# CliMA/ClimateParameterizations.jl

Hardware: AMD Instinct MI355X
Metric: column-timesteps/sec (fwd+adjoint), 32-level wind-mixing NDE (higher is better)
Workload: dtype f32

## Files before the change

### climateparameterizations.jl_amd/csrc/engine_regtile.hip

```cpp
#include <cstdlib>
#include "regtile_dev.h"
#include "kernel_select.h"

#ifndef RT16_WAVES
#define RT16_WAVES 8
#endif
#ifndef RT_ADJ_CH
#define RT_ADJ_CH 8
#endif
#define RT_TAPEZ (20 * 256)
#define RT_TAPE2 (20 * 256)

__host__ __device__ constexpr int rt16_q_net(int Q) { return Q < 36 ? Q / 12 : Q - 36; }
__host__ __device__ constexpr int rt16_q_quad(int Q) { return Q < 36 ? Q % 12 : 12; }
__host__ __device__ constexpr int rt16_q_slot(int n, int qq) { return qq < 12 ? 12 * n + qq : 36 + n; }

template <int ACT>
__device__ __forceinline__ void rt_mlp_forward(const float* wl, const RtBases& b, const f32x16 (&X)[3], int h, f32x16 (&O)[3]) {
    f32x16 A1[5];
#pragma unroll
    for (int mt = 0; mt < 5; mt++) {
        f32x16 acc;
#pragma unroll
        for (int r = 0; r < 16; r++) {
// ... 568 lines not shown
                            for (int G = 0; G < 24; G += 4) rt_act_pair4_at<ACT>(A1, D1, G);
                            rt_act_pair_at<ACT>(A1, D1, 24);
                        }
                    } else {
#pragma unroll
                        for (int t = 0; t < 2; t++) {
                            f32x16 acc;
#pragma unroll
                            for (int r = 0; r < 16; r++) acc[r] = (t * 16 + r < 25) ? wl[RT_B1C + n * 50 + 2 * (t * 16 + r) + h] : 0.0f;
                            const int base = a1n[t] + n * 50 * RT_LD1;
                            acc = rt_chain<48, RT_ADJ_CH>(wl, acc, [=](int k) { return base + (k >> 4) * 32 + RHO0(k & 15); },
                                                          [&](int k) { return X[k >> 4][k & 15]; });
#pragma unroll
                            for (int r = 0; r < 16; r++) {
                                float av = 0.0f, dv = 0.0f;
                                if (t * 16 + r < 25) rt_act_pair<ACT>(acc[r], av, dv);
                                A1[t][r] = av;
                                D1[t][r] = dv;
                            }
                        }
                    }
                    RT_STAMP(1);
                    f32x16 Z2;
                    {
                        f32x16 acc;
#pragma unroll
                        for (int r = 0; r < 16; r++) acc[r] = r < 10 ? wl[RT_B2C + n * 20 + 2 * r + h] : 0.0f;
                        const int base2 = a2b + n * 20 * RT_LD2;
                        Z2 = rt_chain<25, 5>(wl, acc, [=](int k) { return base2 + 2 * k; },
                                             [&](int k) { return A1[k >> 4][k & 15]; });
                    }
                    RT_STAMP(2);
                    {
                        f32x16 TA;
                        if (EARLY3 && n == 0) TA = TA3;
                        else { TA = rt_transpose(tb, dOn, wbase, rbase); b3acc[n] += rt_sum16(TA); }
                        f32x16 A2;
#pragma unroll
                        for (int r = 0; r < 16; r += 4) {
                            f32x2v a0 = {0.0f, 0.0f}, d0 = {0.0f, 0.0f}, a1 = {0.0f, 0.0f}, d1 = {0.0f, 0.0f};
                            if (r < 8) rt_act_pair4<ACT>((f32x2v){Z2[r], Z2[r + 1]}, (f32x2v){Z2[r + 2], Z2[r + 3]}, a0, d0, a1, d1);
                            else if (r == 8) rt_act_pair2<ACT>((f32x2v){Z2[8], Z2[9]}, a0, d0);
                            A2[r] = a0.x; A2[r + 1] = a0.y; A2[r + 2] = a1.x; A2[r + 3] = a1.y;
                            Z2[r] = d0.x; Z2[r + 1] = d0.y; Z2[r + 2] = d1.x; Z2[r + 3] = d1.y;
                        }
                        const f32x16 TB = rt_transpose(tb, A2, wbase, rbase);
                        gW3[n] = rt_outer(gW3[n], TA, TB);
                    }
                    {
                        const int base = b3T + n * 31 * RT_LD3;
                        f32x16 da;
                        if (EARLY3 && n == 0) da = da3;
                        else da = rt_chain<16, 8>(wl, (f32x16)(0.0f), [=](int k) { return base + RHO0(k) * RT_LD3; },
                                                  [&](int k) { return dOn[k]; });
#pragma unroll
                        for (int r = 0; r < 16; r++) Z2[r] = da[r] * Z2[r];
                    }
                    RT_STAMP(3);
                    if (ZT && n < 2) load_z1(step, st, n + 1, A1n);
                    u32x4 Lr[9];
                    const u32x4* lg = nullptr;
                    if constexpr (SPLIT) {
                        int lz = lane;
                        asm volatile("" : "+v"(lz));
                        lg = reinterpret_cast<const u32x4*>(wimg + RT_ASIMG_OFF + RT_ASIMG_L) + n * 9 * 64 + lz;
#pragma unroll
                        for (int u = 0; u < 3; u++) Lr[u] = lg[u * 64];
                    }
                    {
                        const f32x16 TA = rt_transpose(tb, Z2, wbase, rbase);
                        b2acc[n] += rt_sum16(TA);
#pragma unroll
                        for (int t = 0; t < 2; t++) {
                            const f32x16 TB = rt_transpose(tb, A1[t], wbase, rbase);
                            gW2[n][t] = rt_outer(gW2[n][t], TA, TB);
                        }
                    }
                    RT_STAMP(4);
#pragma unroll
                    for (int t = 0; t < 2; t++) {
                        const int base = b2T[t] + n * 20 * RT_LD2;
                        const f32x16 da = rt_chain<10, 10>(wl, (f32x16)(0.0f), [=](int k) { return base + 2 * k * RT_LD2; },
                                                           [&](int k) { return Z2[k]; });
#pragma unroll
                        for (int r = 0; r < 16; r++) D1[t][r] = da[r] * D1[t][r];
                    }
                    auto store_delta = [&] {
#pragma unroll
                    for (int g = 0; g < 25; g++) {
                        const int G = 25 * n + g;
                        if ((G & 3) == 0 && g + 3 < 25) {
                            const f32x4v v = {D1[g >> 4][g & 15], D1[(g + 1) >> 4][(g + 1) & 15], D1[(g + 2) >> 4][(g + 2) & 15],
                                              D1[(g + 3) >> 4][(g + 3) & 15]};
                            RT_NT_STORE4(dst + (G >> 2) * 256, v);
                        }
                    }
                    if (n == 0) carry[0] = D1[1][8];
                    if (n == 1) {
                        RT_NT_STORE4(dst + 6 * 256, ((f32x4v){carry[0], D1[0][0], D1[0][1], D1[0][2]}));
                        carry[0] = D1[1][7];
                        carry[1] = D1[1][8];
                    }
                    if (n == 2) {
                        RT_NT_STORE4(dst + 12 * 256, ((f32x4v){carry[0], carry[1], D1[0][0], D1[0][1]}));
                        RT_NT_STORE4(dst + 18 * 256, ((f32x4v){D1[1][6], D1[1][7], D1[1][8], 0.0f}));
                    }
                    };
                    if constexpr (!SPLIT) store_delta();
                    RT_STAMP(5);
                    if (ZT && n < 2) __builtin_amdgcn_sched_barrier(0);
                    if constexpr (SPLIT) {
                        const u32x4* hm = reinterpret_cast<const u32x4*>(rt_smem) + lane;
#pragma unroll
                        for (int c = 0; c < 3; c++) {
                            if (c < 2) {
#pragma unroll
                                for (int u = 0; u < 3; u++) Lr[3 * (c + 1) + u] = lg[(3 * (c + 1) + u) * 64];
                            }
                            float d8[8];
#pragma unroll
                            for (int u = 0; u < 8; u++) d8[u] = D1[(8 * c + u) >> 4][(8 * c + u) & 15];
                            const Bf3 Bc = bf3_split8(d8);
#pragma unroll
                            for (int q = 0; q < 3; q++) {
                                const int G = n * 9 + c * 3 + q, slot = c * 3 + q;
                                const u32x4 Ah = hm[(G * 2) * 64], Am = hm[(G * 2 + 1) * 64];
                                if (ZT && n < 2 && slot >= 2) {
                                    if (slot == 2) z1_stamp(n);
                                    if (slot < 8) rt_act_pair4_at<ACT>(A1n, D1n, 4 * (slot - 2));
                                    else rt_act_pair_at<ACT>(A1n, D1n, 24);
                                }
                                xb[q] = mfma_bf(Am, Bc.m, xb[q]);
                                xb[q] = mfma_bf(Ah, Bc.l, xb[q]);
                                xb[q] = mfma_bf(Am, Bc.h, xb[q]);
                                xb[q] = mfma_bf(Ah, Bc.m, xb[q]);
                                xb[q] = mfma_bf(Ah, Bc.h, xb[q]);
                                xb[q] = mfma_bf(Lr[slot], Bc.h, xb[q]);
                                RT_SCHED_FENCE();
                            }
                        }
                        const float* left = rt_smem + RT_ASIMG_LEFT + (n * 2 + h) * 96 + i_;
#pragma unroll
                        for (int q = 0; q < 3; q++) xb[q] = mfma32(left[q * 32], D1[1][8], xb[q]);
                        store_delta();
                    } else
#pragma unroll
                    for (int q = 0; q < 3; q++) {
                        const int base = b1T + q * 32 + n * 50 * RT_LD1;
                        xb[q] = rt_chain_fill<25, 5>(wl, xb[q], [=](int g) { return base + 2 * g * RT_LD1; },
                                                     [&](int g) { return D1[g >> 4][g & 15]; },
                                                     [&](int c) {
                                                         if (ZT && n < 2 && (q > 0 || c > 0)) {
                                                             if (q * 5 + c == 2) z1_stamp(n);
#pragma unroll
                                                             for (int G = 0; G < 24; G += 4)
                                                                 if ((G >> 2) * 2 + 2 == q * 5 + c)
                                                                     rt_act_pair4_at<ACT>(A1n, D1n, G);
                                                             if (q * 5 + c == 14) rt_act_pair_at<ACT>(A1n, D1n, 24);
                                                         }
                                                     });
                    }
                    if (ZT && n < 2) {
#pragma unroll
                        for (int t = 0; t < 2; t++) { A1[t] = A1n[t]; D1[t] = D1n[t]; }
                    }
                }
                RT_STAMP(6);
#pragma unroll
                for (int q = 0; q < 3; q++) xbs[q] += xb[q];
            }
#pragma unroll
            for (int q = 0; q < 3; q++) {
#pragma unroll
                for (int r = 0; r < 16; r++) lam[RT_LAM(q * 16 + r, lane)] += xbs[q][r];
                xbs[q] = (f32x16)(0.0f);
            }
        }
    }

#ifndef COLNDE_STAMPS_FWD
    RT_STAMP_FLUSH();
#endif
    float* out = slab + (size_t)tile * (m.n_params + 8);
    const int r_j = (j & 3) + 4 * (j >> 3), h_j = (j >> 2) & 1;
#pragma unroll
    for (int n = 0; n < 3; n++) {
        if (r_j < 10) {
            const int f2 = 2 * r_j + h_j;
#pragma unroll
            for (int r = 0; r < 16; r++) {
                const int face = RHO0(r) + 4 * h;
                if (face >= 1) out[n * m.net_size + m.w_off[2] + f2 * 31 + face - 1] = gW3[n][r];
            }
        }
#pragma unroll
        for (int t = 0; t < 2; t++) {
            const int Gp = t * 16 + r_j;
            if (Gp < 25) {
                const int f1 = 2 * Gp + h_j;
#pragma unroll
                for (int r = 0; r < 10; r++) out[n * m.net_size + m.w_off[1] + f1 * 20 + 2 * r + h] = gW2[n][t][r];
            }
        }
        const float s2 = b2acc[n] + swap32(b2acc[n], h), s3 = b3acc[n] + swap32(b3acc[n], h);
        if (h == 0) {
            if (r_i < 10) out[n * m.net_size + m.b_off[1] + 2 * r_i + h_i] = s2;
            if (i_ >= 1) out[n * m.net_size + m.b_off[2] + i_ - 1] = s3;
        }
    }
#pragma unroll
    for (int q = 0; q < 6; q++) {
        float v = sums[q];
        for (int off = 32; off > 0; off >>= 1) v += __shfl_down(v, off);
        if (lane == 0) out[m.n_params + q] = v;
    }
}

#define RT_DW1_LDS (4 * 2048)
__global__ void __launch_bounds__(256)
rt_dw1_kernel(DevModel m, const float* __restrict__ tape, const float* __restrict__ tape2, long n_items,
              float* __restrict__ slab_rows) {
    const int lane = threadIdx.x & 63, wave = __builtin_amdgcn_readfirstlane(threadIdx.x >> 6);
    const int j = lane & 31, h = lane >> 5;
    float* buf = rt_smem + wave * RT_DW1_LDS;
    const long gw = (long)blockIdx.x * RT_WAVES + wave, GW = (long)gridDim.x * RT_WAVES;
    f32x16 gW1[5][3];
#pragma unroll
    for (int mt = 0; mt < 5; mt++)
#pragma unroll
        for (int q = 0; q < 3; q++) gW1[mt][q] = (f32x16)(0.0f);
    float b1acc[5] = {0, 0, 0, 0, 0};
    const int NQ = gw < n_items ? 4 * (int)((n_items - gw + GW - 1) / GW) : 0;
    const int soff = ((lane >> 1) & 3) * 256 + ((lane & 1) * 32 + (lane >> 3)) * 4;
    auto issue = [&](int Q, int ring) {
        const int Qc = Q < NQ ? Q : NQ - 1;
        const size_t item = (size_t)(gw + (long)(Qc >> 2) * GW);
        const float* sx = tape + item * 3072 + soff + (Qc & 3) * 32;
        const float* sz = tape2 + item * RT_TAPE2 + soff + (Qc & 3) * 32;
#pragma unroll
        for (int T = 0; T < 3; T++) __builtin_amdgcn_global_load_lds(sx + T * 1024, buf + ring * 2048 + T * 256, 16, 0, RT_DMA_AUX);
#pragma unroll
        for (int T = 0; T < 5; T++) __builtin_amdgcn_global_load_lds(sz + T * 1024, buf + ring * 2048 + (3 + T) * 256, 16, 0, RT_DMA_AUX);
    };
    const float* rd = buf + h * 32 + j;
    float op[2][8][4];
    auto read_set = [&](int set, int ring) {
#pragma unroll
        for (int T = 0; T < 8; T++)
#pragma unroll
            for (int s = 0; s < 4; s++) op[set][T][s] = rd[ring * 2048 + T * 256 + 64 * s];
    };
    if (NQ > 0) {
        issue(0, 0);
        issue(1, 1);
        issue(2, 2);
        asm volatile("s_waitcnt vmcnt(16)" ::: "memory");
        read_set(0, 0);
    }
    for (int Qb = 0; Qb < NQ; Qb += 4) {
#pragma unroll
        for (int u = 0; u < 4; u++) {
            const int cur = u & 1;
#pragma unroll
            for (int s = 0; s < 4; s++)
#pragma unroll
                for (int q = 0; q < 3; q++) gW1[0][q] = mfma32(op[cur][3][s], op[cur][q][s], gW1[0][q]);
            b1acc[0] += (op[cur][3][0] + op[cur][3][1]) + (op[cur][3][2] + op[cur][3][3]);
            __builtin_amdgcn_sched_barrier(0);
            issue(Qb + u + 3, (u + 3) & 3);
            asm volatile("s_waitcnt vmcnt(16)" ::: "memory");
            read_set(cur ^ 1, (u + 1) & 3);
            __builtin_amdgcn_sched_barrier(0);
#pragma unroll
            for (int mt = 1; mt < 5; mt++) {
#pragma unroll
                for (int s = 0; s < 4; s++)
#pragma unroll
                    for (int q = 0; q < 3; q++) gW1[mt][q] = mfma32(op[cur][3 + mt][s], op[cur][q][s], gW1[mt][q]);
                b1acc[mt] += (op[cur][3 + mt][0] + op[cur][3 + mt][1]) + (op[cur][3 + mt][2] + op[cur][3 + mt][3]);
            }
            __builtin_amdgcn_sched_barrier(0);
        }
    }
    asm volatile("s_waitcnt vmcnt(0)" ::: "memory");
    float* out = slab_rows + (size_t)gw * (m.n_params + 8);
#pragma unroll
    for (int mt = 0; mt < 5; mt++) {
#pragma unroll
        for (int r = 0; r < 16; r++) {
            const int G = mt * 16 + r;
            if (G < 75) {
                const int n = G / 25, f = 2 * (G % 25) + h;
#pragma unroll
                for (int q = 0; q < 3; q++) out[n * m.net_size + m.w_off[0] + (q * 32 + j) * 50 + f] = gW1[mt][q][r];
            }
        }
        const float s1 = b1acc[mt] + swap32(b1acc[mt], h);
        const int r_j = (j & 3) + 4 * (j >> 3), h_j = (j >> 2) & 1;
        const int G = mt * 16 + r_j;
        if (h == 0 && G < 75) out[(G / 25) * m.net_size + m.b_off[0] + 2 * (G % 25) + h_j] = s1;
    }
}

__global__ void __launch_bounds__(256)
rt_dw1_split_kernel(DevModel m, const float* __restrict__ tape, const float* __restrict__ tape2, long n_items,
                    float* __restrict__ slab_rows) {
    const int lane = threadIdx.x & 63, wave = __builtin_amdgcn_readfirstlane(threadIdx.x >> 6);
    const int j = lane & 31, h = lane >> 5;
    float* buf = rt_smem + wave * RT_DW1_LDS;
    const long gw = (long)blockIdx.x * RT_WAVES + wave, GW = (long)gridDim.x * RT_WAVES;
    f32x16 gW1[5][3];
#pragma unroll
    for (int mt = 0; mt < 5; mt++)
#pragma unroll
        for (int q = 0; q < 3; q++) gW1[mt][q] = (f32x16)(0.0f);
    float b1acc[5] = {0, 0, 0, 0, 0};
    const int NQ = gw < n_items ? 4 * (int)((n_items - gw + GW - 1) / GW) : 0;
    const int soff = ((lane >> 1) & 3) * 256 + ((lane & 1) * 32 + (lane >> 3)) * 4;
    auto issue = [&](int Q, int ring) {
        const int Qc = Q < NQ ? Q : NQ - 1;
        const size_t item = (size_t)(gw + (long)(Qc >> 2) * GW);
        const float* sx = tape + item * 3072 + soff + (Qc & 3) * 32;
        const float* sz = tape2 + item * RT_TAPE2 + soff + (Qc & 3) * 32;
#pragma unroll
        for (int T = 0; T < 3; T++) __builtin_amdgcn_global_load_lds(sx + T * 1024, buf + ring * 2048 + T * 256, 16, 0, RT_DMA_AUX);
#pragma unroll
        for (int T = 0; T < 5; T++) __builtin_amdgcn_global_load_lds(sz + T * 1024, buf + ring * 2048 + (3 + T) * 256, 16, 0, RT_DMA_AUX);
    };
    const float* rd = buf + h * 2048 + j;
    float raw[2][8][8];
    auto read_half = [&](int set, int slot0) {
#pragma unroll
        for (int T = 0; T < 8; T++)
#pragma unroll
            for (int c = 0; c < 8; c++) raw[set][T][c] = rd[slot0 * 2048 + T * 256 + c * 32];
    };
    if (NQ > 0) {
        issue(0, 0);
        issue(1, 1);
        issue(2, 2);
        issue(3, 3);
        asm volatile("s_waitcnt vmcnt(16)" ::: "memory");
        read_half(0, 0);
        asm volatile("s_waitcnt lgkmcnt(0)" ::: "memory");
        issue(4, 0);
        issue(5, 1);
    }
    for (int Qb = 0; Qb < NQ; Qb += 4) {
#pragma unroll
        for (int u = 0; u < 2; u++) {
            const int cur = u;
            asm volatile("s_waitcnt vmcnt(16)" ::: "memory");
            read_half(cur ^ 1, 2 * (u ^ 1));
            __builtin_amdgcn_sched_barrier(0);
            Bf3 X[3];
#pragma unroll
            for (int q = 0; q < 3; q++) X[q] = bf3_split8(raw[cur][q]);
            __builtin_amdgcn_sched_barrier(0);
            asm volatile("s_waitcnt lgkmcnt(0)" ::: "memory");
            issue(Qb + 2 * u + 6, 2 * (u ^ 1));
            issue(Qb + 2 * u + 7, 2 * (u ^ 1) + 1);
            __builtin_amdgcn_sched_barrier(0);
#pragma unroll
            for (int mt = 0; mt < 5; mt++) {
                const Bf3 Z = bf3_split8(raw[cur][3 + mt]);
#pragma unroll
                for (int q = 0; q < 3; q++) gW1[mt][q] = mfma_bf3(Z, X[q], gW1[mt][q]);
                const float* z = raw[cur][3 + mt];
                b1acc[mt] += ((z[0] + z[1]) + (z[2] + z[3])) + ((z[4] + z[5]) + (z[6] + z[7]));
            }
            __builtin_amdgcn_sched_barrier(0);
        }
    }
    asm volatile("s_waitcnt vmcnt(0)" ::: "memory");
    float* out = slab_rows + (size_t)gw * (m.n_params + 8);
#pragma unroll
    for (int mt = 0; mt < 5; mt++) {
#pragma unroll
        for (int r = 0; r < 16; r++) {
            const int G = mt * 16 + r;
            if (G < 75) {
                const int n = G / 25, f = 2 * (G % 25) + h;
#pragma unroll
                for (int q = 0; q < 3; q++) out[n * m.net_size + m.w_off[0] + (q * 32 + j) * 50 + f] = gW1[mt][q][r];
            }
        }
        const float s1 = b1acc[mt] + swap32(b1acc[mt], h);
        const int r_j = (j & 3) + 4 * (j >> 3), h_j = (j >> 2) & 1;
        const int G = mt * 16 + r_j;
        if (h == 0 && G < 75) out[(G / 25) * m.net_size + m.b_off[0] + 2 * (G % 25) + h_j] = s1;
    }
}

template <int ACT, bool SPLIT = false>
__global__ void __launch_bounds__(512)
rt16_forward_kernel(DevModel m, const float* __restrict__ wimg, const float* __restrict__ x0, const float* __restrict__ bcs,
                    const float* __restrict__ save_times, int n_save, int substeps, float* __restrict__ sol,
                    float* __restrict__ tape, float* __restrict__ tapez, int n_col) {
    float* wl = rt_smem;
    const float* bl = wl;
    const u32x4* simg = reinterpret_cast<const u32x4*>(rt_smem);
    if constexpr (SPLIT) {
        const unsigned* src = reinterpret_cast<const unsigned*>(wimg + RT_SIMG_OFF);
        unsigned* dst = reinterpret_cast<unsigned*>(rt_smem);
        for (int e = threadIdx.x; e < RT_SIMG_WORDS / 4; e += blockDim.x)
            reinterpret_cast<u32x4*>(dst)[e] = reinterpret_cast<const u32x4*>(src)[e];
        for (int e = threadIdx.x; e < RT_IMG_FLOATS - RT_B1C; e += blockDim.x) wl[RT_SIMG_WORDS + e] = wimg[RT_B1C + e];
        bl = wl + RT_SIMG_WORDS - RT_B1C;
    } else {
        for (int e = threadIdx.x; e < RT_IMG_FLOATS; e += blockDim.x) wl[e] = wimg[e];
    }
    __syncthreads();
    const int lane = threadIdx.x & 63, wave = threadIdx.x >> 6;
    const int j = lane & 15, g = lane >> 4;
    const int wt = blockIdx.x * (blockDim.x >> 6) + wave;
    const int tile32 = wt >> 1, half = wt & 1;
    if (tile32 * 32 >= n_col) return;
    const int col = wt * 16 + j;
    const bool valid = col < n_col;
    const int colc = min(col, n_col - 1);
    const int i_ = lane & 15, g_i = i_ >> 2, r_i = i_ & 3;
    int a1b[10];
#pragma unroll
    for (int t = 0; t < 10; t++) {
        const int Q = 4 * t + r_i, f = 4 * rt16_q_quad(Q) + g_i;
        const int row = (Q < 39 && f < 50) ? rt16_q_net(Q) * 50 + f : 0;
        a1b[t] = RT_W1C + row * RT_LD1 + 4 * g;
    }
    int a2b[2], a2l[2], a3b[2];
#pragma unroll
    for (int u = 0; u < 2; u++) {
        const int Q2 = 4 * u + r_i;
        const int row2 = Q2 < 5 ? 4 * Q2 + g_i : 0;
        a2b[u] = RT_W2C + row2 * RT_LD2 + g;
        a2l[u] = RT_W2C + row2 * RT_LD2 + (g < 2 ? 48 + g : 50);
        a3b[u] = RT_W3C + (16 * u + i_ - 1) * RT_LD3 + g;
    }
    RtBC bc;
    float bc5;
    {
        const float* bp = bcs + (size_t)colc * 6;
        bc.b[0] = bp[0]; bc.t[0] = bp[1]; bc.b[1] = bp[2]; bc.t[1] = bp[3]; bc.b[2] = bp[4]; bc5 = bp[5];
        bc.t[2] = bc5;
    }
    V16 Xn[3];
#pragma unroll
    for (int q = 0; q < 3; q++)
#pragma unroll
        for (int tau = 0; tau < 2; tau++) {
            const f32x4v v = *reinterpret_cast<const f32x4v*>(x0 + (size_t)colc * 96 + q * 32 + 16 * tau + 4 * g);
            Xn[q].t[tau] = v;
            if (sol && valid) *reinterpret_cast<f32x4v*>(sol + ((size_t)col * n_save) * 96 + q * 32 + 16 * tau + 4 * g) = v;
        }
    const int n_steps = (n_save - 1) * substeps;
    RT_STAMP_DECL;
#ifdef COLNDE_STAMPS_FWD
    const unsigned long long rs_k0 = __builtin_amdgcn_s_memtime(), rs_r0 = __builtin_amdgcn_s_memrealtime();
#endif
    float* tp = tape ? tape + (size_t)tile32 * n_steps * 4 * 3072 + ((g >> 1) * 64 + j + 16 * half + 32 * (g & 1)) * 4 : nullptr;
    float* tz = tapez ? tapez + (size_t)tile32 * n_steps * 4 * RT_TAPEZ + ((g >> 1) * 64 + j + 16 * half + 32 * (g & 1)) * 4 : nullptr;
    const float Nz = 32.0f;
    struct { float cU, sU, cV, sV, cB, sB, kE, oE, cE, nA, nB, f0, f1, f2; } pc;
    {
        const float L2E = 1.4426950408889634f;
        pc.cU = m.sig_u * Nz; pc.sU = m.sig_u * m.eps; pc.cV = m.sig_v * Nz; pc.sV = m.sig_v * m.eps; pc.cB = m.B * Nz; pc.sB = m.B * m.eps;
        pc.kE = 2.0f * m.inv_dRi * L2E; pc.oE = -2.0f * m.Ric * m.inv_dRi * L2E; pc.cE = 30.0f * L2E;
        pc.nA = -0.5f * m.nu_minus; pc.nB = m.nu0 + 0.5f * m.nu_minus;
        pc.f0 = -m.cs[0] * Nz; pc.f1 = -m.cs[1] * Nz; pc.f2 = -m.cs[2] * m.inv_Pr * Nz;
    }
    int step = 0;
    for (int iv = 0; iv < n_save - 1; iv++) {
        const float t0 = save_times[iv];
        const float dt = (save_times[iv + 1] - t0) / (float)substeps;
        for (int s = 0; s < substeps; s++, step++) {
            const float ts = t0 + (float)s * dt;
            V16 Xs[3], Kacc[3];
#pragma unroll
            for (int q = 0; q < 3; q++) { Xs[q] = Xn[q]; Kacc[q].t[0] = (f32x4t)(0.0f); Kacc[q].t[1] = (f32x4t)(0.0f); }
#pragma nounroll
            for (int st = 0; st < 4; st++) {
                const float ca = st == 0 ? 0.0f : (st == 3 ? 1.0f : 0.5f);
                const float cb = (st == 0 || st == 3) ? 1.0f / 6.0f : 1.0f / 3.0f;
                RT_STAMP_BEGIN();
                if (tp) {
                    float* o = tp + ((size_t)step * 4 + st) * 3072;
#pragma unroll
                    for (int q = 0; q < 3; q++)
#pragma unroll
                        for (int tau = 0; tau < 2; tau++) *reinterpret_cast<f32x4v*>(o + (q * 4 + 2 * tau) * 256) = Xs[q].t[tau];
                }
                bc.t[2] = rt_top_flux(m, bc5, ts + ca * dt);
                RT_STAMP(0);
                f32x4t A1[10];
                int lz = lane;
                if constexpr (SPLIT) asm volatile("" : "+v"(lz));
                if constexpr (SPLIT) {
#pragma unroll
                    for (int t = 0; t < 10; t++)
#pragma unroll
                        for (int r = 0; r < 4; r++) {
                            const int Q = 4 * t + r;
                            A1[t][r] = Q < 39 ? bl[RT_B1C + rt16_q_net(Q) * 50 + min(4 * rt16_q_quad(Q) + g, 49)] : 0.0f;
                        }
                    Bf3 Apf = rt16_ldA(simg, 0, lz);
#pragma unroll
                    for (int q = 0; q < 3; q++) {
                        const float x8[8] = {Xs[q].t[0][0], Xs[q].t[0][1], Xs[q].t[0][2], Xs[q].t[0][3], Xs[q].t[1][0], Xs[q].t[1][1], Xs[q].t[1][2], Xs[q].t[1][3]};
                        const Bf3 XB = bf3_split8(x8);
#pragma unroll
                        for (int t = 0; t < 10; t++) {
                            const Bf3 Ac = Apf;
                            const int nx = q * 10 + t + 1;
                            if (nx < 30) Apf = rt16_ldA(simg, 3 * (nx % 10) + nx / 10, lz);
                            auto finish = [&](int tt) {
                                float* oz = tz ? tz + ((size_t)step * 4 + st) * RT_TAPEZ + 2 * tt * 256 : nullptr;
                                if (tz) *reinterpret_cast<f32x4v*>(oz) = A1[tt];
#pragma unroll
                                for (int r = 0; r < 4; r++) asm volatile("" : "+v"(A1[tt][r]));
                                A1[tt] = rt_act4<ACT, false>(A1[tt]);
#pragma unroll
                                for (int r = 0; r < 4; r++) asm volatile("" : "+v"(A1[tt][r]));
                            };
                            if (q == 2) RT_SCHED_HARD();
                            __builtin_amdgcn_s_setprio(1);
                            A1[t] = mfma16_bf3(Ac, XB, A1[t]);
                            __builtin_amdgcn_s_setprio(0);
                            if (q == 2) {
                                if (t > 0) {
                                    finish(t - 1);
#pragma unroll
                                    for (int u = 0; u < 6; u++) {
                                        __builtin_amdgcn_sched_group_barrier(0x008, 1, 0);
                                        __builtin_amdgcn_sched_group_barrier(0x402, 9, 0);
                                    }
                                }
                                RT_SCHED_HARD();
                                if (t == 9) finish(9);
                            } else
                                RT_SCHED_FENCE();
                        }
                    }
                } else {
                auto finish1 = [&](int tt) {
                    float* oz = tz ? tz + ((size_t)step * 4 + st) * RT_TAPEZ + 2 * tt * 256 : nullptr;
                    if (tz) *reinterpret_cast<f32x4v*>(oz) = A1[tt];
#pragma unroll
                    for (int r = 0; r < 4; r++) asm volatile("" : "+v"(A1[tt][r]));
                    A1[tt] = rt_act4<ACT>(A1[tt]);
#pragma unroll
                    for (int r = 0; r < 4; r++) asm volatile("" : "+v"(A1[tt][r]));
                };
#pragma unroll
                for (int t = 0; t < 10; t++) {
                    f32x4t acc;
#pragma unroll
                    for (int r = 0; r < 4; r++) {
                        const int Q = 4 * t + r;
                        acc[r] = Q < 39 ? wl[RT_B1C + rt16_q_net(Q) * 50 + min(4 * rt16_q_quad(Q) + g, 49)] : 0.0f;
                    }
                    const int base = a1b[t];
                    acc = rt16_chain<24, 8>(wl, acc, [=](int k) { return base + (k >> 3) * 32 + ((k >> 2) & 1) * 16 + (k & 3); },
                                            [&](int k) { return Xs[k >> 3].t[(k >> 2) & 1][k & 3]; });
                    A1[t] = acc;
                    finish1(t);
                }
                }
                RT_STAMP(1);
                V16 O[3];
#pragma unroll
                for (int n = 0; n < 3; n++) {
                    f32x4t A2[2];
                    Bf3 HB[2];
                    if constexpr (SPLIT) {
#pragma unroll
                        for (int c = 0; c < 2; c++) {
                            float a8[8];
#pragma unroll
                            for (int e = 0; e < 8; e++) a8[e] = 8 * c + e < 13 ? A1[rt16_q_slot(n, 8 * c + e) >> 2][rt16_q_slot(n, 8 * c + e) & 3] : 0.0f;
                            HB[c] = bf3_split8(a8);
                        }
                    }
#pragma unroll
                    for (int u = 0; u < 2; u++) {
                        f32x4t acc;
#pragma unroll
                        for (int r = 0; r < 4; r++) acc[r] = (4 * u + r < 5) ? bl[RT_B2C + n * 20 + 4 * (4 * u + r) + g] : 0.0f;
                        if constexpr (SPLIT) {
                            const Bf3 Aa = rt16_ldA(simg, 30 + 4 * n + 2 * u, lz), Ab = rt16_ldA(simg, 30 + 4 * n + 2 * u + 1, lz);
                            __builtin_amdgcn_s_setprio(1);
                            acc = mfma16_bf3(Aa, HB[0], acc);
                            acc = mfma16_bf3(Ab, HB[1], acc);
                            __builtin_amdgcn_s_setprio(0);
                            RT_SCHED_FENCE();
                        } else {
                        const int base = a2b[u] + n * 20 * RT_LD2, basel = a2l[u] + n * 20 * RT_LD2;
                        acc = rt16_chain<13, 13>(wl, acc, [=](int k) { return k < 12 ? base + 4 * k : basel; },
                                                 [&](int k) { return A1[rt16_q_slot(n, k) >> 2][rt16_q_slot(n, k) & 3]; });
                        }
                        A2[u] = SPLIT && u == 0 ? rt_act4<ACT, false>(acc) : rt_act4<ACT>(acc);
                    }
                    Bf3 GB;
                    if constexpr (SPLIT) {
                        const float a8[8] = {A2[0][0], A2[0][1], A2[0][2], A2[0][3], A2[1][0], 0.0f, 0.0f, 0.0f};
                        GB = bf3_split8(a8);
                    }
#pragma unroll
                    for (int v = 0; v < 2; v++) {
                        f32x4t acc;
#pragma unroll
                        for (int r = 0; r < 4; r++) acc[r] = bl[RT_B3C + n * 32 + 16 * v + 4 * g + r];
                        if constexpr (SPLIT) {
                            const Bf3 Aa = rt16_ldA(simg, 42 + 2 * n + v, lz);
                            __builtin_amdgcn_s_setprio(1);
                            O[n].t[v] = mfma16_bf3(Aa, GB, acc);
                            __builtin_amdgcn_s_setprio(0);
                            RT_SCHED_FENCE();
                        } else {
                        const int base = a3b[v] + n * 31 * RT_LD3;
                        O[n].t[v] = rt16_chain<5, 5>(wl, acc, [=](int k) { return base + 4 * k; },
                                                     [&](int k) { return A2[k >> 2][k & 3]; });
                        }
                    }
                }
                RT_STAMP(2);
                V16 F[3];
                {
                    V16 Ud, Vd, Td;
                    if (m.mpp || m.ca) {
                        Ud = shift_down16(Xs[0], lane, 0.0f); Vd = shift_down16(Xs[1], lane, 0.0f); Td = shift_down16(Xs[2], lane, 0.0f);
                    }
                    if (m.mpp) {
                        if constexpr (SPLIT) {
#pragma unroll
                            for (int tau = 0; tau < 2; tau++)
#pragma unroll
                                for (int r = 0; r < 4; r++) {
#pragma clang fp contract(off)
                                    const float dU = Xs[0].t[tau][r] - Ud.t[tau][r], dV = Xs[1].t[tau][r] - Vd.t[tau][r], dT = Xs[2].t[tau][r] - Td.t[tau][r];
                                    const float a1 = fmaf(dU, pc.cU, pc.sU), a2 = fmaf(dV, pc.cV, pc.sV);
                                    const float rS = __builtin_amdgcn_rcpf(fmaf(a1, a1, a2 * a2));
                                    const float arg = fmaf(fmaf(dT, pc.cB, pc.sB) * rS, pc.kE, pc.oE);
                                    const float e = __builtin_amdgcn_exp2f(__builtin_amdgcn_fmed3f(arg, -pc.cE, pc.cE));
                                    const float rc = __builtin_amdgcn_rcpf(e + 1.0f);
                                    const float nu = fmaf(fmaf(rc, -2.0f, 1.0f), pc.nA, pc.nB);
                                    F[0].t[tau][r] = fmaf(nu * dU, pc.f0, O[0].t[tau][r]);
                                    F[1].t[tau][r] = fmaf(nu * dV, pc.f1, O[1].t[tau][r]);
                                    F[2].t[tau][r] = fmaf(nu * dT, pc.f2, O[2].t[tau][r]);
                                }
                        } else
#pragma unroll
                        for (int tau = 0; tau < 2; tau++)
#pragma unroll
                            for (int r = 0; r < 4; r += 2) {
                                const f32x2v dU = {Xs[0].t[tau][r] - Ud.t[tau][r], Xs[0].t[tau][r + 1] - Ud.t[tau][r + 1]};
                                const f32x2v dV = {Xs[1].t[tau][r] - Vd.t[tau][r], Xs[1].t[tau][r + 1] - Vd.t[tau][r + 1]};
                                const f32x2v dT = {Xs[2].t[tau][r] - Td.t[tau][r], Xs[2].t[tau][r + 1] - Td.t[tau][r + 1]};
                                const f32x2v a1 = dU * pc.cU + pc.sU, a2 = dV * pc.cV + pc.sV;
                                const f32x2v s2 = a2 * a2 + a1 * a1;
                                f32x2v rS;
                                rS.x = __builtin_amdgcn_rcpf(s2.x);
                                rS.y = __builtin_amdgcn_rcpf(s2.y);
                                const f32x2v arg = ((dT * pc.cB + pc.sB) * rS) * pc.kE + pc.oE;
                                f32x2v e;
                                e.x = __builtin_amdgcn_exp2f(__builtin_amdgcn_fmed3f(arg.x, -pc.cE, pc.cE));
                                e.y = __builtin_amdgcn_exp2f(__builtin_amdgcn_fmed3f(arg.y, -pc.cE, pc.cE));
                                const f32x2v e1 = e + 1.0f;
                                f32x2v rc;
                                rc.x = __builtin_amdgcn_rcpf(e1.x);
                                rc.y = __builtin_amdgcn_rcpf(e1.y);
                                const f32x2v nu = (rc * -2.0f + 1.0f) * pc.nA + pc.nB;
                                const f32x2v o0 = {O[0].t[tau][r], O[0].t[tau][r + 1]}, o1 = {O[1].t[tau][r], O[1].t[tau][r + 1]},
                                             o2 = {O[2].t[tau][r], O[2].t[tau][r + 1]};
                                const f32x2v f0 = (nu * dU) * pc.f0 + o0, f1 = (nu * dV) * pc.f1 + o1, f2 = (nu * dT) * pc.f2 + o2;
                                F[0].t[tau][r] = f0.x; F[0].t[tau][r + 1] = f0.y;
                                F[1].t[tau][r] = f1.x; F[1].t[tau][r + 1] = f1.y;
// ... 181 lines not shown
```

Before: 203.1 million.

## Software-pipeline dW1 split kernel by interleaving MFMAs with LDS reads, DMA and bf16 splits

Restructures the dW1 accumulation loop into a compile-time scheduled pipeline. Each MFMA slot is interleaved with a measured share of VALU work: splitting the next Z and X tiles into bf16 triples, the bias-sum adds, LDS reads of the next half, and global-to-LDS DMA issues. Z and X splits are double-buffered across iterations, and DMA addresses are advanced incrementally instead of recomputed. The goal is to hide VALU and memory latency behind the matrix cores, at the cost of much more complex code, higher register pressure, and fragile hand-placed waitcnts.

```diff
diff --git a/climateparameterizations.jl_amd/csrc/engine_regtile.hip b/climateparameterizations.jl_amd/csrc/engine_regtile.hip
--- a/climateparameterizations.jl_amd/csrc/engine_regtile.hip
+++ b/climateparameterizations.jl_amd/csrc/engine_regtile.hip
@@ -894,6 +894,57 @@
     }
 }
 
+template <class F, int... I>
+__device__ __forceinline__ void rt_static_for_(F&& f, std::integer_sequence<int, I...>) { (f(std::integral_constant<int, I>{}), ...); }
+template <int N, class F>
+__device__ __forceinline__ void rt_static_for(F&& f) { rt_static_for_(f, std::make_integer_sequence<int, N>{}); }
+
+constexpr int dw1_nx(int p) { return p < 4 ? 2 : 4; }
+constexpr int dw1_nx_before(int p) { return 2 * p; }
+constexpr int dw1_nvalu(int p) { return 44 + 8 + 11 * dw1_nx(p); }
+constexpr bool dw1_read_gap(int p, int g) { return p < 4 && g < 8; }
+constexpr bool dw1_dma_gap(int p, int g) { return p < 4 && g >= 9 && g <= 15 && (g & 1); }
+constexpr int dw1_room(int p, int g) { return 6 - (dw1_read_gap(p, g) ? 1 : dw1_dma_gap(p, g) ? 3 : 0); }
+constexpr int dw1_room_before(int p, int g) { int s = 0; for (int i = 0; i < g; i++) s += dw1_room(p, i); return s; }
+constexpr int dw1_op_begin(int p, int g) { return dw1_nvalu(p) * dw1_room_before(p, g) / dw1_room_before(p, 18); }
+
+struct Dw1Tmp { float ha, hb, ra, rb, la, lb, s0, s1, s2, s3; };
+
+template <int K>
+__device__ __forceinline__ void dw1_split_op(float a, float b, int pp, Dw1Tmp& t, Bf3& o) {
+    if constexpr (K == 0) t.ha = __uint_as_float(__float_as_uint(a) & 0xffff0000u);
+    if constexpr (K == 1) t.ra = a - t.ha;
+    if constexpr (K == 2) t.hb = __uint_as_float(__float_as_uint(b) & 0xffff0000u);
+    if constexpr (K == 3) t.rb = b - t.hb;
+    if constexpr (K == 4) o.h[pp] = __builtin_amdgcn_perm(__float_as_uint(b), __float_as_uint(a), 0x07060302u);
+    if constexpr (K == 5) t.ha = __uint_as_float(__float_as_uint(t.ra) & 0xffff0000u);
+    if constexpr (K == 6) t.la = t.ra - t.ha;
+    if constexpr (K == 7) t.hb = __uint_as_float(__float_as_uint(t.rb) & 0xffff0000u);
+    if constexpr (K == 8) t.lb = t.rb - t.hb;
+    if constexpr (K == 9) o.m[pp] = __builtin_amdgcn_perm(__float_as_uint(t.rb), __float_as_uint(t.ra), 0x07060302u);
+    if constexpr (K == 10) o.l[pp] = __builtin_amdgcn_perm(__float_as_uint(t.lb), __float_as_uint(t.la), 0x07060302u);
+}
+template <int K>
+__device__ __forceinline__ void dw1_b1_op(const float* z, Dw1Tmp& t, float& b) {
+    if constexpr (K == 0) t.s0 = z[0] + z[1];
+    if constexpr (K == 1) t.s1 = z[2] + z[3];
+    if constexpr (K == 2) t.s2 = z[4] + z[5];
+    if constexpr (K == 3) t.s3 = z[6] + z[7];
+    if constexpr (K == 4) t.s0 = t.s0 + t.s1;
+    if constexpr (K == 5) t.s2 = t.s2 + t.s3;
+    if constexpr (K == 6) t.s0 = t.s0 + t.s2;
+    if constexpr (K == 7) b += t.s0;
+}
+template <int K>
+__device__ __forceinline__ sp_f32x16 dw1_product(const Bf3& a, const Bf3& b, sp_f32x16 c) {
+    if constexpr (K == 0) return mfma_bf(a.m, b.m, c);
+    if constexpr (K == 1) return mfma_bf(a.l, b.h, c);
+    if constexpr (K == 2) return mfma_bf(a.h, b.l, c);
+    if constexpr (K == 3) return mfma_bf(a.m, b.h, c);
+    if constexpr (K == 4) return mfma_bf(a.h, b.m, c);
+    if constexpr (K == 5) return mfma_bf(a.h, b.h, c);
+}
+
 __global__ void __launch_bounds__(256)
 rt_dw1_split_kernel(DevModel m, const float* __restrict__ tape, const float* __restrict__ tape2, long n_items,
                     float* __restrict__ slab_rows) {
@@ -927,6 +978,16 @@
 #pragma unroll
             for (int c = 0; c < 8; c++) raw[set][T][c] = rd[slot0 * 2048 + T * 256 + c * 32];
     };
+    auto piece = [&](const float* qx, const float* qz, int ring, int T) {
+        const float* src = (T < 3 ? qx + T * 1024 : qz + (T - 3) * 1024) + soff;
+        __builtin_amdgcn_global_load_lds(src, buf + ring * 2048 + T * 256, 16, 0, RT_DMA_AUX);
+    };
+    const int NI = NQ >> 2;
+    const size_t sx = (size_t)GW * 3072, sz = (size_t)GW * RT_TAPE2;
+    const size_t lx = (size_t)(gw + (long)(NI - 1) * GW) * 3072, lz = (size_t)(gw + (long)(NI - 1) * GW) * RT_TAPE2;
+    size_t ax = NI > 1 ? (size_t)(gw + GW) * 3072 : lx, az = NI > 1 ? (size_t)(gw + GW) * RT_TAPE2 : lz;
+    Bf3 X[2][3], Zt[2];
+    Dw1Tmp tmp;
     if (NQ > 0) {
         issue(0, 0);
         issue(1, 1);
@@ -937,32 +998,54 @@
         asm volatile("s_waitcnt lgkmcnt(0)" ::: "memory");
         issue(4, 0);
         issue(5, 1);
-    }
+        __builtin_amdgcn_sched_barrier(0);
+#pragma unroll
+        for (int q = 0; q < 3; q++) X[0][q] = bf3_split8(raw[0][q]);
+        Zt[0] = bf3_split8(raw[0][3]);
+        __builtin_amdgcn_sched_barrier(0);
+        asm volatile("s_waitcnt vmcnt(16)" ::: "memory");
+    }
+    auto half = [&](auto U) {
+        constexpr int u = decltype(U)::value, nx = u ^ 1;
+        const size_t qx0 = ax + (2 - 2 * u) * 32, qx1 = qx0 + 32, qz0 = az + (2 - 2 * u) * 32, qz1 = qz0 + 32;
+        rt_static_for<5>([&](auto Pp) {
+            constexpr int p = decltype(Pp)::value, zc = (5 * u + p) & 1, zn = zc ^ 1;
+            rt_static_for<18>([&](auto Gg) {
+                constexpr int g = decltype(Gg)::value;
+                if constexpr (p == 4 && g == 0) asm volatile("s_waitcnt vmcnt(16)" ::: "memory");
+                gW1[p][g / 6] = dw1_product<g % 6>(Zt[zc], X[u][g / 6], gW1[p][g / 6]);
+                if constexpr (dw1_read_gap(p, g)) {
+                    constexpr int T = 2 * p + g / 4, k = g % 4;
+                    raw[nx][T][2 * k] = rd[2 * nx * 2048 + T * 256 + 2 * k * 32];
+                    raw[nx][T][2 * k + 1] = rd[2 * nx * 2048 + T * 256 + (2 * k + 1) * 32];
+                }
+                if constexpr (dw1_dma_gap(p, g)) {
+                    constexpr int d = (g - 9) / 2;
+                    if constexpr (d == 0) asm volatile("s_waitcnt lgkmcnt(0)" ::: "memory");
+                    piece(tape + ((d & 1) ? qx1 : qx0), tape2 + ((d & 1) ? qz1 : qz0), 2 * nx + (d & 1), 2 * p + (d >> 1));
+                }
+                rt_static_for<dw1_op_begin(p, g + 1) - dw1_op_begin(p, g)>([&](auto Ii) {
+                    constexpr int i = dw1_op_begin(p, g) + decltype(Ii)::value;
+                    if constexpr (i < 44) {
+                        const float* z = raw[p < 4 ? u : nx][p < 4 ? 4 + p : 3];
+                        dw1_split_op<i % 11>(z[2 * (i / 11)], z[2 * (i / 11) + 1], i / 11, tmp, Zt[zn]);
+                    } else if constexpr (i < 52) {
+                        dw1_b1_op<i - 44>(raw[u][3 + p], tmp, b1acc[p]);
+                    } else {
+                        constexpr int pr = dw1_nx_before(p) + (i - 52) / 11;
+                        const float* x = raw[nx][pr / 4];
+                        dw1_split_op<(i - 52) % 11>(x[2 * (pr % 4)], x[2 * (pr % 4) + 1], pr % 4, tmp, X[nx][pr / 4]);
+                    }
+                });
+                __builtin_amdgcn_sched_barrier(0);
+            });
+        });
+    };
     for (int Qb = 0; Qb < NQ; Qb += 4) {
-#pragma unroll
-        for (int u = 0; u < 2; u++) {
-            const int cur = u;
-            asm volatile("s_waitcnt vmcnt(16)" ::: "memory");
-            read_half(cur ^ 1, 2 * (u ^ 1));
-            __builtin_amdgcn_sched_barrier(0);
-            Bf3 X[3];
-#pragma unroll
-            for (int q = 0; q < 3; q++) X[q] = bf3_split8(raw[cur][q]);
-            __builtin_amdgcn_sched_barrier(0);
-            asm volatile("s_waitcnt lgkmcnt(0)" ::: "memory");
-            issue(Qb + 2 * u + 6, 2 * (u ^ 1));
-            issue(Qb + 2 * u + 7, 2 * (u ^ 1) + 1);
-            __builtin_amdgcn_sched_barrier(0);
-#pragma unroll
-            for (int mt = 0; mt < 5; mt++) {
-                const Bf3 Z = bf3_split8(raw[cur][3 + mt]);
-#pragma unroll
-                for (int q = 0; q < 3; q++) gW1[mt][q] = mfma_bf3(Z, X[q], gW1[mt][q]);
-                const float* z = raw[cur][3 + mt];
-                b1acc[mt] += ((z[0] + z[1]) + (z[2] + z[3])) + ((z[4] + z[5]) + (z[6] + z[7]));
-            }
-            __builtin_amdgcn_sched_barrier(0);
-        }
+        half(std::integral_constant<int, 0>{});
+        ax = ax + sx < lx ? ax + sx : lx;
+        az = az + sz < lz ? az + sz : lz;
+        half(std::integral_constant<int, 1>{});
     }
     asm volatile("s_waitcnt vmcnt(0)" ::: "memory");
     float* out = slab_rows + (size_t)gw * (m.n_params + 8);
```

After: 203.5 million (median of 6 runs). Within noise of the previous version (+0.2%).
